# posgraph/coupe.DVSG

Measured on AMD Instinct MI355X. Metric: stabilized frames/sec (1280x720 RGB), higher is better.
Workload: dtype f32

## Files before the change

### coupe/dvsg_amd/_lib.py

```python
import ctypes
import os

_HERE = os.path.dirname(os.path.abspath(__file__))
LIB_PATH = os.environ.get("DVSG_AMD_LIB") or os.path.join(_HERE, "libdvsg_amd.so")
ABI_VERSION = 1

c_float_p = ctypes.POINTER(ctypes.c_float)
_vp = ctypes.c_void_p
_i = ctypes.c_int

SIGNATURES = {
    "dvsg_tps_solve_f32": [_vp, _vp, _i, _i, _i, _vp, _vp],
    "dvsg_tps_solve_checked_f32": [_vp, _vp, _i, _i, _i, _vp, _vp, _vp],
    "dvsg_tps_warp_f32": [_vp, _vp, _vp, _i, _i, _i, _i, _i, _i, _i, _vp, _vp, _vp, _vp],
    "dvsg_flow_warp_f32": [_vp, _vp, _i, _i, _i, _i, _vp, _vp],
    "dvsg_stn_sample_f32": [_vp, _vp, _vp, _i, _i, _i, _i, _i, _i, _vp, _vp],
    "dvsg_grid_affine_f32": [_vp, _vp, _i, _i, _i, _i, _i, _i, _vp, _vp, _vp, _vp],
    "dvsg_grid_projective_f32": [_vp, _vp, _i, _i, _i, _i, _i, _i, _vp, _vp, _vp, _vp],
    "dvsg_elastic_constants_f32": [_i, _vp, _vp],
    "dvsg_grid_elastic_f32": [_vp, _vp, _vp, _i, _vp, _i, _i, _i, _i, _i, _i, _vp, _vp, _vp, _vp],
    "dvsg_scale_rgb_f32": [_vp, _i, _i, _i, _i, _vp, _vp],
    "dvsg_locnet_create": [_i, ctypes.POINTER(ctypes.c_char_p), ctypes.POINTER(_vp),
                           ctypes.POINTER(_i), ctypes.POINTER(ctypes.c_int64), ctypes.POINTER(_vp)],
    "dvsg_locnet_destroy": [_vp],
# ... 51 lines not shown
QUERIES = ("dvsg_abi_version", "dvsg_last_error_string", "dvsg_target_arch")

_lib = None


class DvsgError(RuntimeError):
    pass


def load():
    global _lib
    if _lib is not None:
        return _lib
    if not os.path.isfile(LIB_PATH):
        raise DvsgError(
            "libdvsg_amd.so not found at %s: build it with ./build.sh (hipcc --offload-arch=gfx950). "
            "coupe.dvsg_amd has no CPU or PyTorch fallback." % LIB_PATH)
    lib = ctypes.CDLL(LIB_PATH)
    lib.dvsg_abi_version.restype = ctypes.c_int
    lib.dvsg_last_error_string.restype = ctypes.c_char_p
    lib.dvsg_target_arch.restype = ctypes.c_char_p
    if lib.dvsg_abi_version() != ABI_VERSION:
        raise DvsgError("libdvsg_amd.so ABI %d != expected %d" % (lib.dvsg_abi_version(), ABI_VERSION))
    for name, argtypes in SIGNATURES.items():
        fn = getattr(lib, name)
        fn.argtypes = argtypes
        fn.restype = ctypes.c_int
    _lib = lib
    for env, opt in (("DVSG_CONV_VARIANT", b"conv_variant"), ("DVSG_FUSE_CONV", b"fuse_conv"),
                     ("DVSG_F16_SPLIT", b"f16_split"), ("DVSG_FUSE_SHORTCUT", b"fuse_shortcut"),
                     ("DVSG_CONV1_VARIANT", b"conv1_variant"), ("DVSG_F16_PAIR_MASK", b"f16_pair_mask"),
                     ("DVSG_WIDE16_PACKED", b"wide16_packed"), ("DVSG_WIDE16_AROWS", b"wide16_arows"),
                     ("DVSG_WIDE16_HREUSE", b"wide16_hreuse"), ("DVSG_FUSED_HREUSE", b"fused_hreuse"),
                     ("DVSG_CONCAT_SC", b"concat_sc"), ("DVSG_FLOW_TILED", b"flow_tiled")):
        if os.environ.get(env) and os.environ.get("DVSG_DEBUG") == "1":
            check(lib.dvsg_debug_set_option(opt, int(os.environ[env])), "dvsg_debug_set_option")
    return lib


def check(status, what):
    if status != 0:
        msg = load().dvsg_last_error_string().decode("utf-8", "replace")
        raise DvsgError("%s failed (status %d): %s" % (what, status, msg))


def call(name, *args):
    check(getattr(load(), name)(*args), name)
```

### coupe/dvsg_amd/csrc/cnn_kernels.h

```cpp
#pragma once
#include "common.h"

namespace dvsg {

enum Precision { kF32 = 0, kF16 = 1, kF32S = 2, kF32X = 3 };
inline size_t elem_size(int prec) { return prec == kF16 ? 2 : 4; }

struct ConvGemm {
  int prec;
  const void *x;
  const void *wt;
  const float *bias;
  const void *res;
  void *y;
  int B, H, W, Cin, Ho, Wo, Cout;
  int ksize, stride, pad;
  int res_H, res_W, res_stride;
  int relu;
  int ldx = 0, res_ld = 0, relu_from = -1;
  const void *wt_packed = nullptr;
  const void *wt_packed_a = nullptr;
  const void *wt_packed_h = nullptr;
  int x3 = 0;
  int wsplit = 0;
// ... 11 lines not shown
size_t wide16_packed_bytes(int rows, int Cin, int ksize);
int launch_pack_wide16(const void *wt, void *out, int rows, int Cin, int ksize, int order, hipStream_t s);
void set_wide16_arows(int v);
void set_wide16_hreuse(int v);
void set_wide16_packed(int v);
int launch_zero_tickets(int *tickets, size_t n, hipStream_t s);
struct ConvFused {
  const float *x;
  const float *wt2;
  const float *bias2;
  const float *wt3;
  const float *bias3;
  const float *res;
  float *y;
  int B, H, W, Cin, Ho, Wo, Cout;
  int stride;
  int res_H, res_W, res_stride;
  const float *sc_x = nullptr;
  const float *sc_wt = nullptr;
  const float *sc_bias = nullptr;
  int sc_cin = 0;
  int pieces = 0;
  int f16 = 0;
  int x3 = 0;
};
int launch_conv3x3_1x1_x3(const ConvFused &p, hipStream_t s);
bool conv_fusable(int prec, int Cin, int Cmid, int Cout, int ksize);
int launch_conv3x3_1x1(const ConvFused &p, hipStream_t s);
void set_fuse_conv(int v);
int get_fuse_conv();
void set_fused_hreuse(int v);
void set_conv_variant(int v);
void set_conv1_variant(int v);

constexpr int kConv1Cin = 21;
constexpr int kConv1K = 7 * kConv1Cin;
constexpr int kConv1Kpad = 148;
constexpr int kConv1Ld = 150;
constexpr int kConv1LdH = 168;
constexpr int kConv1X3Ld = 88;
constexpr int kConv1X3StageElems = 3 * 64 * kConv1X3Ld;
enum Conv1SrcKind { kSrcWindow = 0, kSrcRingF32 = 1, kSrcRingU8 = 2 };
struct Conv1Src {
  const void *base;
  const int *table;
  int n_pool;
  const float *mask = nullptr;
};
int launch_conv1(int out_prec, const Conv1Src &src, int src_kind, const float *wt1, const void *wt1h, const void *wt1s,
                 const void *wt1x, const float *bias, void *y, int B, int H, int W, int Ho, int Wo, hipStream_t s);

int launch_maxpool(int prec, const void *x, void *y, int B, int H, int W, int C, int Ho, int Wo, int pad_top,
                   int pad_left, hipStream_t s);

constexpr int kPoolSplits = 8;
int launch_avgpool_partial(int prec, const void *x, float *part, int B, int HW, int C, hipStream_t s);

int launch_f16_to_f32(const void *x, float *y, size_t n, hipStream_t s);
int launch_p_to_f32(const void *x, float *y, size_t n, hipStream_t s);
int launch_f32_to_p(const float *x, void *y, size_t n, hipStream_t s);

constexpr int kDenseSplits = 8;
int launch_dense(const float *xin, int s_in, const float *bias_in, float scale_in, int lrelu_in,
                 const float *W, float *out_part, int B, int K, int N, hipStream_t s);
int launch_dense_finalize(const float *part, int s_in, float scale, const float *bias, float *out, int B,
                          int N, hipStream_t s);

}
```

### coupe/dvsg_amd/csrc/conv1_pool.hip

```cpp
#include <cstdint>
#include <type_traits>

#include "cnn_device.h"
#include "cnn_kernels.h"

namespace dvsg {
namespace {

constexpr int C1_TILE = 128;
constexpr int C1_SEG_PAD = 5488;
constexpr int C1_WELEMS = 64 * kConv1Ld;
constexpr int C1_LDC = 68;

template <int NT, int GROUPS, bool ALIGNED, bool MASKED = false>
struct Conv1Row {
  static constexpr bool kRing = false;
  typedef float floatx4_u __attribute__((ext_vector_type(4), aligned(4)));
  floatx4 nmean[GROUPS];
  long idx[GROUPS];
  unsigned col_ok, full;
  bool fast;
  struct Data {
    floatx4 reg[GROUPS];
    float m0[MASKED ? GROUPS : 1], m1[MASKED ? GROUPS : 1];
// ... 425 lines not shown
  const unsigned long long t_loop_end = C1_STAMP();
#endif
  float *Cs = w_s;
  __syncthreads();
#pragma unroll
  for (int mi = 0; mi < MI; ++mi)
#pragma unroll
    for (int q = 0; q < 16; ++q)
      Cs[(wm * 32 * MI + mi * 32 + (q & 3) + 8 * (q >> 2) + 4 * h) * C1_LDC + wn * 32 + r] = acc[mi][q];
  __syncthreads();
  const int col4 = tid & 15, row0 = tid >> 4;
  const float4 b4 = *reinterpret_cast<const float4 *>(bias + 4 * col4);
  TO *yrow = y + (((size_t)b * Ho + ho) * Wo + wo0) * 64 + 4 * col4;
#pragma unroll 4
  for (int row = row0; row < C1_TILE; row += NT / 16) {
    if (wo0 + row >= Wo) break;
    float4 v = *reinterpret_cast<const float4 *>(Cs + row * C1_LDC + 4 * col4);
    v.x = fmaxf(v.x + b4.x, 0.f);
    v.y = fmaxf(v.y + b4.y, 0.f);
    v.z = fmaxf(v.z + b4.z, 0.f);
    v.w = fmaxf(v.w + b4.w, 0.f);
    store4(yrow + (size_t)row * 64, v);
  }
#ifdef DVSG_STAMPS
  if (tid == 0 && blockIdx.x < 65536) {
    unsigned long long *o = g_c1_stamps + (size_t)blockIdx.x * 8;
    const unsigned long long t_end = C1_STAMP();
    o[0] = st[0]; o[1] = st[1]; o[2] = st[2]; o[3] = st[3]; o[4] = st[4];
    o[5] = t_loop_end - t_begin;
    o[6] = t_end - t_begin;
    o[7] = __builtin_amdgcn_s_memrealtime() - r_begin;
  }
#endif
}

template <typename T>
__global__ __launch_bounds__(256) void maxpool_kernel(const T *__restrict__ x, T *__restrict__ y, int H, int W,
                                                     int C4, int Ho, int Wo, int pad_top, int pad_left,
                                                     size_t total) {
  {
    const size_t e = (size_t)xcd_remap(blockIdx.x, gridDim.x) * 256 + threadIdx.x;
    if (e >= total) return;
    const int c4 = (int)(e % C4);
    size_t t = e / C4;
    const int wo = (int)(t % Wo);
    t /= Wo;
    const int ho = (int)(t % Ho);
    const size_t b = t / Ho;
    float4 m = make_float4(-INFINITY, -INFINITY, -INFINITY, -INFINITY);
#pragma unroll
    for (int i = 0; i < 3; ++i) {
      const int hi = 2 * ho - pad_top + i;
      if (hi < 0 || hi >= H) continue;
#pragma unroll
      for (int j = 0; j < 3; ++j) {
        const int wi = 2 * wo - pad_left + j;
        if (wi < 0 || wi >= W) continue;
        const float4 v = load4(x + (((b * H + hi) * W + wi) * C4 + c4) * 4);
        m.x = fmaxf(m.x, v.x);
        m.y = fmaxf(m.y, v.y);
        m.z = fmaxf(m.z, v.z);
        m.w = fmaxf(m.w, v.w);
      }
    }
    store4(y + e * 4, m);
  }
// ... 964 lines not shown
    if (hi < 0 || hi >= H) continue;
#pragma unroll
    for (int j = 0; j < 3; ++j) {
      const int wi = 2 * wo - pad_left + j;
      if (wi < 0 || wi >= W) continue;
      const float4 v = load4_p(x, (((b * H + hi) * W + wi) * C4 + c4) * 4);
      m.x = fmaxf(m.x, v.x);
      m.y = fmaxf(m.y, v.y);
      m.z = fmaxf(m.z, v.z);
      m.w = fmaxf(m.w, v.w);
    }
  }
  store4_p(y, e * 4, m);
}

int march_bands(int B, int Ho, int wtiles, int *quads_per_band) {
  const int quads = (Ho + C1M_QUAD - 1) / C1M_QUAD;
  const long cols = (long)B * wtiles;
  for (int qpb = 8; qpb >= 4; --qpb) {
    const int bands = (quads + qpb - 1) / qpb;
    if (cols * bands >= 3 * 256) {
      if (quads_per_band) *quads_per_band = qpb;
      return bands;
    }
  }
  return 0;
}

int g_conv1_variant = 0;

}

void set_conv1_variant(int v) { g_conv1_variant = v; }

int launch_conv1(int out_prec, const Conv1Src &src, int src_kind, const float *wt1, const void *wt1h, const void *wt1s,
                 const void *wt1x, const float *bias, void *y, int B, int H, int W, int Ho, int Wo, hipStream_t s) {
  const int wtiles = ceil_div(Wo, C1_TILE);
  const long blocks = (long)wtiles * Ho * B;
  DVSG_REQUIRE(blocks > 0 && blocks < (1L << 31), "conv1: grid of %ld workgroups out of range", blocks);
  DVSG_REQUIRE((long)W * kConv1Cin < (1L << 31), "conv1: input row too long");
  DVSG_REQUIRE(src_kind == kSrcWindow || (src.table && src.n_pool > 0), "conv1: a frame ring needs its index table");
  const double in_bytes = src_kind == kSrcRingU8 ? 1.0 : 4.0;
  ProfScope prof(kClsConv1, s, 2.0 * (double)B * Ho * Wo * 64 * 49 * kConv1Cin,
                 in_bytes * (double)B * H * W * kConv1Cin + (double)elem_size(out_prec) * B * Ho * Wo * 64);
  const dim3 grid((unsigned)blocks);
  const bool aligned = W % 4 == 0 && reinterpret_cast<uintptr_t>(src.base) % (src_kind == kSrcRingU8 ? 4 : 16) == 0;
  const int SRC = 2 * src_kind + (aligned ? 1 : 0) + (src.mask ? 8 : 0);
  if (out_prec == kF32S && !wt1s) return fail(DVSG_ERR_UNSUPPORTED, "conv1: the f32s precision needs the piece weights");
#define DVSG_K_F32(SRC) conv1_kernel<4, float, SRC>
#define DVSG_K_F16(SRC) conv1_f16_kernel<_Float16, (SRC) & 7>
#define DVSG_K_SPLIT(SRC) conv1_split_kernel<float, SRC>
#define DVSG_K_X3(SRC) conv1_x3_kernel<SRC>
#define DVSG_C1(KERNEL, NTHREADS, WPTR, YPTR)                                                                            \
  do {                                                                                                                   \
    switch (SRC) {                                                                                                       \
      case 0: hipLaunchKernelGGL((KERNEL(0)), grid, dim3(NTHREADS), 0, s, src, WPTR, bias, YPTR, H, W, Ho, Wo, wtiles); break; \
      case 1: hipLaunchKernelGGL((KERNEL(1)), grid, dim3(NTHREADS), 0, s, src, WPTR, bias, YPTR, H, W, Ho, Wo, wtiles); break; \
      case 2: hipLaunchKernelGGL((KERNEL(2)), grid, dim3(NTHREADS), 0, s, src, WPTR, bias, YPTR, H, W, Ho, Wo, wtiles); break; \
      case 3: hipLaunchKernelGGL((KERNEL(3)), grid, dim3(NTHREADS), 0, s, src, WPTR, bias, YPTR, H, W, Ho, Wo, wtiles); break; \
      case 4: hipLaunchKernelGGL((KERNEL(4)), grid, dim3(NTHREADS), 0, s, src, WPTR, bias, YPTR, H, W, Ho, Wo, wtiles); break; \
      case 5: hipLaunchKernelGGL((KERNEL(5)), grid, dim3(NTHREADS), 0, s, src, WPTR, bias, YPTR, H, W, Ho, Wo, wtiles); break; \
      case 8: hipLaunchKernelGGL((KERNEL(8)), grid, dim3(NTHREADS), 0, s, src, WPTR, bias, YPTR, H, W, Ho, Wo, wtiles); break; \
      case 9: hipLaunchKernelGGL((KERNEL(9)), grid, dim3(NTHREADS), 0, s, src, WPTR, bias, YPTR, H, W, Ho, Wo, wtiles); break; \
      case 10: hipLaunchKernelGGL((KERNEL(10)), grid, dim3(NTHREADS), 0, s, src, WPTR, bias, YPTR, H, W, Ho, Wo, wtiles); break; \
      case 11: hipLaunchKernelGGL((KERNEL(11)), grid, dim3(NTHREADS), 0, s, src, WPTR, bias, YPTR, H, W, Ho, Wo, wtiles); break; \
      case 12: hipLaunchKernelGGL((KERNEL(12)), grid, dim3(NTHREADS), 0, s, src, WPTR, bias, YPTR, H, W, Ho, Wo, wtiles); break; \
// ... 63 lines not shown
#undef DVSG_K_X3
  return check_launch("conv1_kernel");
}

#ifdef DVSG_STAMPS
extern "C" int dvsg_debug_read_conv1_stamps(void *host, size_t bytes) {
  return hipMemcpyFromSymbol(host, HIP_SYMBOL(g_c1_stamps), bytes) == hipSuccess ? 0 : -3;
}
#endif

int launch_maxpool(int prec, const void *x, void *y, int B, int H, int W, int C, int Ho, int Wo, int pad_top,
                   int pad_left, hipStream_t s) {
  DVSG_REQUIRE(C % 4 == 0 && (prec != kF32S || C % 32 == 0), "maxpool: C=%d must be a multiple of 4 (32 in the f32s format)", C);
  const size_t total = (size_t)B * Ho * Wo * (C / 4);
  const size_t want = (total + 255) / 256;
  DVSG_REQUIRE(want < (1u << 31), "maxpool: %zu blocks do not fit a grid", want);
  const int blocks = (int)want;
  ProfScope prof(kClsMaxpool, s, 0.0, (double)elem_size(prec) * C * ((double)B * H * W + (double)B * Ho * Wo));
  if (prec == kF32S)
    hipLaunchKernelGGL(maxpool_p_kernel, dim3(blocks), dim3(256), 0, s, x, y, H, W, C / 4, Ho, Wo, pad_top, pad_left, total);
  else if (prec == kF16 && C % 8 == 0) {
    const size_t total8 = total / 2;
    hipLaunchKernelGGL(maxpool_h8_kernel, dim3((unsigned)((total8 + 255) / 256)), dim3(256), 0, s, static_cast<const _Float16 *>(x),
                       static_cast<_Float16 *>(y), H, W, C / 8, Ho, Wo, pad_top, pad_left, total8);
  } else if (prec == kF16)
    hipLaunchKernelGGL(maxpool_kernel<_Float16>, dim3(blocks), dim3(256), 0, s, static_cast<const _Float16 *>(x),
                       static_cast<_Float16 *>(y), H, W, C / 4, Ho, Wo, pad_top, pad_left, total);
  else
    hipLaunchKernelGGL(maxpool_kernel<float>, dim3(blocks), dim3(256), 0, s, static_cast<const float *>(x),
                       static_cast<float *>(y), H, W, C / 4, Ho, Wo, pad_top, pad_left, total);
  return check_launch("maxpool_kernel");
}

}
```

### coupe/dvsg_amd/csrc/locnet.hip

```cpp
#include <cmath>
#include <cstring>
#include <map>
#include <string>
#include <vector>

#include "cnn_kernels.h"

namespace dvsg {
namespace {

constexpr float kBnEps = 1e-5f;
const char *kPrefix = "stabNet/localizationNet/";

struct HostArray {
  const float *data;
  int nd;
  int64_t dims[4];
  size_t size() const {
    size_t n = 1;
    for (int i = 0; i < nd; ++i) n *= (size_t)dims[i];
    return n;
  }
};

// ... 248 lines not shown
  if (int rc = upload(net, wts, &L->wt32s)) return rc;
  if (int rc = upload(net, wtx, &L->wt3x)) return rc;
  return upload(net, shift, &L->bias);
}

struct Dims {
  int H1, W1, Hp, Wp, pad_top, pad_left;
};

Dims root_dims(int H, int W) {
  Dims d;
  d.H1 = (H - 1) / 2 + 1;
  d.W1 = (W - 1) / 2 + 1;
  d.Hp = (d.H1 + 1) / 2;
  d.Wp = (d.W1 + 1) / 2;
  const int pth = std::max((d.Hp - 1) * 2 + 3 - d.H1, 0), ptw = std::max((d.Wp - 1) * 2 + 3 - d.W1, 0);
  d.pad_top = pth / 2;
  d.pad_left = ptw / 2;
  return d;
}

size_t align256(size_t n) { return (n + 255) & ~(size_t)255; }

int g_f16_split = 1;
int g_f16_pair_mask = 0xFFFF;
enum LayerKind { kKindC1 = 0, kKindC2 = 1, kKindC3 = 2, kKindSc = 3 };
inline bool f16_pairs(const dvsg_locnet *net, int block, int kind) {
  return g_f16_split && ((g_f16_pair_mask & net->f16_pair_mask) >> (4 * kind + block)) & 1;
}
int g_fuse_shortcut = 1;
int g_x3_conv1 = 1;
int g_x3_fuse = 3;
int g_concat_sc = 1;

struct Workspace {
  char *bufA, *bufB, *bufS, *r1, *r2;
  float *pool_part, *dpart0, *dpart1, *T, *Ft;
  char *splitk_slabs;
  int *splitk_counters;
  size_t total;
};
constexpr int kMaxConvLaunches = 64;

Workspace plan(char *base, int B, int H, int W) {
  const Dims d = root_dims(H, W);
  size_t big_el = std::max((size_t)d.H1 * d.W1 * 64, (size_t)d.Hp * d.Wp * 64);
  size_t small_el = 0;
  {
    int h = d.Hp, w = d.Wp;
    for (const BlockSpec &bs : kBlocks)
      for (int u = 1; u <= bs.units; ++u) {
        const int stride = u == bs.units ? bs.last_stride : 1;
        const int ho = (h - 1) / stride + 1, wo = (w - 1) / stride + 1;
        small_el = std::max(small_el, (size_t)h * w * bs.base);
        big_el = std::max(big_el, (size_t)ho * wo * bs.base * 4);
        if (u == 1) big_el = std::max(big_el, (size_t)h * w * bs.base * 5);
        h = ho; w = wo;
      }
  }
  const size_t big = align256((size_t)B * big_el * sizeof(float));
  const size_t small = align256((size_t)B * small_el * sizeof(float));
  Workspace w;
  size_t off = 0;
  auto take = [&](size_t bytes) {
    char *p = base + off;
    off += align256(bytes);
    return p;
  };
  w.bufA = take(big);
  w.bufB = take(big);
  w.bufS = take(big);
  w.r1 = take(small);
  w.r2 = take(small);
  w.pool_part = reinterpret_cast<float *>(take((size_t)kPoolSplits * B * 2048 * sizeof(float)));
  w.dpart0 = reinterpret_cast<float *>(take((size_t)kDenseSplits * 16 * 2048 * sizeof(float)));
  w.dpart1 = reinterpret_cast<float *>(take((size_t)kDenseSplits * 16 * 2048 * sizeof(float)));
  w.T = reinterpret_cast<float *>(take((size_t)B * 2 * 28 * sizeof(float)));
  w.Ft = reinterpret_cast<float *>(take((size_t)B * 50 * sizeof(float)));
  w.splitk_slabs = take(kSplitKSlabBytes);
  w.splitk_counters = reinterpret_cast<int *>(take((size_t)kMaxConvLaunches * kSplitKMaxTiles * sizeof(int)));
  w.total = off;
  return w;
}

int run_conv(int prec, const ConvLayer &L, bool pairs, const void *x, int B, int H, int W, void *y, int Ho, int Wo,
             const void *res, int res_H, int res_W, int res_stride, bool relu, const Workspace &ws, int *launch_idx,
             hipStream_t s, int ldx = 0, int res_ld = 0, int relu_from = -1) {
  ConvGemm p;
  p.ldx = ldx; p.res_ld = res_ld; p.relu_from = relu_from;
  p.splitk_scratch = ws.splitk_slabs;
  p.splitk_scratch_bytes = kSplitKSlabBytes;
  p.splitk_counters = ws.splitk_counters + (size_t)((*launch_idx)++ % kMaxConvLaunches) * kSplitKMaxTiles;
  p.prec = prec == kF32S || prec == kF32X ? kF32 : prec;
  p.wsplit = prec == kF32S || (prec == kF16 && pairs);
  p.x3 = prec == kF32X;
  if (prec == kF32X && !L.wt3x)
    return fail(DVSG_ERR_UNSUPPORTED, "f32x3: layer %d -> %d (k = %d) has no packed bfloat16 pieces (K %% 32, Cout %% 64)", L.cin, L.cout, L.ksize);
  p.x = x; p.wt = L.weights(prec, p.wsplit != 0); p.bias = L.bias; p.res = res; p.y = y;
  if (prec == kF16 && pairs) {
    p.wt_packed = L.wt16p;
    p.wt_packed_a = L.wt16pa;
// ... 57 lines not shown
    return fail(DVSG_ERR_WORKSPACE, "locnet forward: workspace %zu bytes < required %zu", workspace_bytes, ws.total);
  const Dims d = root_dims(H, W);
  const int gprec = prec;
  if (prec == kF32X) prec = kF32;

  auto tap = [&](int stage, const void *act, int h, int w, int c) -> int {
    if (stage != stop_stage) return 0;
    const size_t n = (size_t)B * h * w * c;
    if (n * sizeof(float) > act_out_bytes)
      return fail(DVSG_ERR_INVALID_ARG, "tap buffer %zu bytes < %zu", act_out_bytes, n * sizeof(float));
    if (prec == kF16) {
      if (int rc = launch_f16_to_f32(act, act_out, n, s)) return rc;
    } else if (prec == kF32S) {
      if (int rc = launch_p_to_f32(act, act_out, n, s)) return rc;
    } else {
      DVSG_HIP(hipMemcpyAsync(act_out, act, n * sizeof(float), hipMemcpyDeviceToDevice, s));
    }
    act_dims[0] = h; act_dims[1] = w; act_dims[2] = c;
    return 1;
  };
#define DVSG_TAP(stage, act, h, w, c)          \
  do {                                         \
    int t_ = tap(stage, act, h, w, c);         \
    if (t_ < 0) return t_;                     \
    if (t_ > 0) return DVSG_OK;                \
  } while (0)
#define DVSG_RUN(call)             \
  do {                             \
    if (int rc_ = (call)) return rc_; \
  } while (0)

  DVSG_RUN(launch_zero_tickets(ws.splitk_counters, (size_t)kMaxConvLaunches * kSplitKMaxTiles, s));
  int launch_idx = 0;
  {
  MarkerRange mr("dvsg/conv1");
  DVSG_RUN(launch_conv1(gprec == kF32X && g_x3_conv1 ? kF32X : prec, src, src_kind, net->conv1.wt, net->conv1.wt16, net->conv1.wt32s,
                        net->conv1.wt3x, net->conv1.bias, ws.bufA, B, H, W, d.H1, d.W1, s));
  }
  DVSG_TAP(0, ws.bufA, d.H1, d.W1, 64);
  {
  MarkerRange mr("dvsg/pool1");
  DVSG_RUN(launch_maxpool(prec, ws.bufA, ws.bufB, B, d.H1, d.W1, 64, d.Hp, d.Wp, d.pad_top, d.pad_left, s));
  }
  DVSG_TAP(1, ws.bufB, d.Hp, d.Wp, 64);

  char *X = ws.bufB, *Y = ws.bufA;
  int h = d.Hp, w = d.Wp;
  int stage = 2;
  int unit_in_block = 0, last_block = -1;
  for (const Unit &u : net->units) {
    unit_in_block = u.block == last_block ? unit_in_block + 1 : 1;
    last_block = u.block;
    char range_name[40];
    std::snprintf(range_name, sizeof(range_name), "dvsg/block%d/unit_%d", u.block + 1, unit_in_block);
    MarkerRange mr(range_name);
    const int ho = (h - 1) / u.stride + 1, wo = (w - 1) / u.stride + 1;
    const void *res = X;
    int res_h = h, res_w = w, res_stride = u.stride;
    const int calib_slot = 3 * (stage - 2);
    DVSG_RUN(calib_record(calib_slot, X, (long)B * h * w, u.c1.cin, s));
    const bool x3_fused = gprec == kF32X && g_x3_fuse == 3;
    const bool x3_unfused = gprec == kF32X && (g_x3_fuse == 0 || (g_x3_fuse == 1 && !u.has_shortcut));
    const bool fuse23 = !x3_unfused && conv_fusable(prec, u.c2.cin, u.c2.cout, u.c3.cout, u.c2.ksize) &&
                        (prec != kF16 || (f16_pairs(net, u.block, kKindC2) && f16_pairs(net, u.block, kKindC3) &&
                                          (!u.has_shortcut || f16_pairs(net, u.block, kKindSc))));
    const bool fuse_sc = fuse23 && !x3_fused && u.has_shortcut && u.stride == 1 && u.shortcut.cin == 64 && u.shortcut.cout == 256 &&
                         g_fuse_shortcut;
    const bool cat = u.has_shortcut && !fuse_sc && u.has_cat && prec != kF16 && g_concat_sc && !g_calib.on && u.stride == 1;
    const void *c2_in = ws.r1;
    int c2_ldx = 0, res_ld = 0;
    if (cat) {
      DVSG_RUN(run_conv(gprec, u.cat, false, X, B, h, w, ws.bufS, h, w, nullptr, 0, 0, 1, false, ws, &launch_idx, s, 0, 0,
                        u.shortcut.cout));
      res = ws.bufS;
      res_h = ho; res_w = wo; res_stride = 1;
// ... 461 lines not shown
  }
  if (std::strcmp(name, "wide16_arows") == 0) {
    set_wide16_arows(value);
    return DVSG_OK;
  }
  if (std::strcmp(name, "wide16_packed") == 0) {
    set_wide16_packed(value);
    return DVSG_OK;
  }
  if (std::strcmp(name, "flow_tiled") == 0) {
    set_flow_tiled(value);
    return DVSG_OK;
  }
  if (std::strcmp(name, "flow_rounds") == 0) {
    set_flow_rounds(value);
    return DVSG_OK;
  }
  if (std::strcmp(name, "warp_xcd") == 0) {
    set_warp_xcd(value);
    return DVSG_OK;
  }
  if (std::strcmp(name, "conv1_variant") == 0) {
    set_conv1_variant(value);
    return DVSG_OK;
  }
  if (std::strcmp(name, "fuse_conv") == 0) {
    set_fuse_conv(value);
    return DVSG_OK;
  }
  if (std::strcmp(name, "concat_sc") == 0) {
    g_concat_sc = value != 0;
    return DVSG_OK;
  }
  if (std::strcmp(name, "x3_conv1") == 0) {
    g_x3_conv1 = value;
    return DVSG_OK;
  }
  if (std::strcmp(name, "x3_fuse") == 0) {
    g_x3_fuse = value;
    return DVSG_OK;
  }
  if (std::strcmp(name, "fuse_shortcut") == 0) {
    g_fuse_shortcut = value != 0;
    return DVSG_OK;
  }
  if (std::strcmp(name, "f16_split") == 0) {
    g_f16_split = value != 0;
    return DVSG_OK;
  }
  if (std::strcmp(name, "f16_pair_mask") == 0) {
    g_f16_pair_mask = value & 0xFFFF;
    return DVSG_OK;
  }
  return fail(DVSG_ERR_INVALID_ARG, "dvsg_debug_set_option: unknown option %s", name);
}

static int calibrate_f16(dvsg_locnet *net, const float *patches, int B, int H, int W, int mode, void *workspace,
                         size_t workspace_bytes, hipStream_t s) {
  std::vector<double> mu((size_t)48 * 2048, 1.0);
  if (mode == 2) {
    void *sums = nullptr, *part = nullptr, *F = nullptr;
    hipError_t e = hipMalloc(&sums, 48 * 2048 * sizeof(double));
    if (e == hipSuccess) e = hipMalloc(&part, (size_t)kCalibBlocks * 2048 * sizeof(float));
    if (e == hipSuccess) e = hipMalloc(&F, (size_t)B * 50 * sizeof(float));
    if (e == hipSuccess) e = hipMemsetAsync(sums, 0, 48 * 2048 * sizeof(double), s);
    int rc = e == hipSuccess ? DVSG_OK : fail(DVSG_ERR_HIP, "calibration: %s", hipGetErrorString(e));
// ... 185 lines not shown
```

Baseline: 743.8.

## Fuse conv1 with 3x3/2 maxpool via banded tiles and seam fixup kernel

Adds a conv1 kernel that max-pools its output tile in shared memory before writing, so the full-resolution conv1 activation never goes to global memory. There are single-group and paired-group (512-thread) variants. Each workgroup covers a band of pooled rows and a strip of columns. Partial maxima at band and strip edges go to side buffers, and a small seams kernel merges them afterwards. With default settings the fused path runs only for f32 conv1, window sources without a mask, and large enough grids; otherwise the separate conv1 and maxpool path is kept. The cost is an extra launch and recomputed boundary rows.

Result: faster. 752.3 (median of 6 runs) (+1.1%).

```diff
diff --git a/coupe/dvsg_amd/_lib.py b/coupe/dvsg_amd/_lib.py
--- a/coupe/dvsg_amd/_lib.py
+++ b/coupe/dvsg_amd/_lib.py
@@ -107,7 +107,9 @@
                      ("DVSG_CONV1_VARIANT", b"conv1_variant"), ("DVSG_F16_PAIR_MASK", b"f16_pair_mask"),
                      ("DVSG_WIDE16_PACKED", b"wide16_packed"), ("DVSG_WIDE16_AROWS", b"wide16_arows"),
                      ("DVSG_WIDE16_HREUSE", b"wide16_hreuse"), ("DVSG_FUSED_HREUSE", b"fused_hreuse"),
-                     ("DVSG_CONCAT_SC", b"concat_sc"), ("DVSG_FLOW_TILED", b"flow_tiled")):
+                     ("DVSG_CONCAT_SC", b"concat_sc"), ("DVSG_FLOW_TILED", b"flow_tiled"),
+                     ("DVSG_CONV1_POOL_FUSED", b"conv1_pool_fused"), ("DVSG_CONV1_POOL_BAND", b"conv1_pool_band"),
+                     ("DVSG_CONV1_POOL_PAIR", b"conv1_pool_pair")):
         if os.environ.get(env) and os.environ.get("DVSG_DEBUG") == "1":
             check(lib.dvsg_debug_set_option(opt, int(os.environ[env])), "dvsg_debug_set_option")
     return lib
diff --git a/coupe/dvsg_amd/csrc/cnn_kernels.h b/coupe/dvsg_amd/csrc/cnn_kernels.h
--- a/coupe/dvsg_amd/csrc/cnn_kernels.h
+++ b/coupe/dvsg_amd/csrc/cnn_kernels.h
@@ -67,6 +67,7 @@
 void set_fused_hreuse(int v);
 void set_conv_variant(int v);
 void set_conv1_variant(int v);
+int get_conv1_variant();
 
 constexpr int kConv1Cin = 21;
 constexpr int kConv1K = 7 * kConv1Cin;
@@ -85,6 +86,10 @@
 int launch_conv1(int out_prec, const Conv1Src &src, int src_kind, const float *wt1, const void *wt1h, const void *wt1s,
                  const void *wt1x, const float *bias, void *y, int B, int H, int W, int Ho, int Wo, hipStream_t s);
 
+void conv1_pool_geometry(int B, int Hp, int Wp, int pband, int *strips, int *bands, size_t *side_elems);
+int launch_conv1_pool(const Conv1Src &src, int src_kind, const float *wt1, const float *bias, float *y, float *side, int B, int H,
+                      int W, int H1, int W1, int Hp, int Wp, int pad_top, int pad_left, int pband, bool pair, hipStream_t s);
+
 int launch_maxpool(int prec, const void *x, void *y, int B, int H, int W, int C, int Ho, int Wo, int pad_top,
                    int pad_left, hipStream_t s);
 
diff --git a/coupe/dvsg_amd/csrc/conv1_pool.hip b/coupe/dvsg_amd/csrc/conv1_pool.hip
--- a/coupe/dvsg_amd/csrc/conv1_pool.hip
+++ b/coupe/dvsg_amd/csrc/conv1_pool.hip
@@ -481,6 +481,423 @@
     o[7] = __builtin_amdgcn_s_memrealtime() - r_begin;
   }
 #endif
+}
+
+constexpr int C1P_Q = C1_TILE / 2;
+constexpr int C1P_TOP = C1P_Q + 1;
+
+template <int SRC>
+__global__ __launch_bounds__(256) __attribute__((amdgpu_waves_per_eu(2, 2)))
+void conv1_pool_kernel(const Conv1Src src, const float *__restrict__ wt1, const float *__restrict__ bias,
+                       float *__restrict__ y, float *__restrict__ side_top, float *__restrict__ side_left, int H, int W,
+                       int H1, int W1, int Hp, int Wp, int pad_top, int pad_left, int strips, int bands, int pband) {
+  constexpr int NT = 256;
+  constexpr int MI = 2;
+  constexpr int IN4 = (C1_SEG_PAD / 4 + NT - 1) / NT;
+  constexpr int WLOADS = (C1_WELEMS / 4 + NT - 1) / NT;
+  const int ROWS = 2 * pband;
+  static_assert(C1_TILE * C1_LDC <= C1_WELEMS, "pool tile must fit in the weight stage");
+  __shared__ __attribute__((aligned(16))) float w_s[C1_WELEMS];
+  __shared__ __attribute__((aligned(16))) float in_s[C1_SEG_PAD];
+  const int tid = threadIdx.x;
+  const int lane = tid & 63, wave = tid >> 6;
+  const int wm = wave >> 1, wn = wave & 1;
+  const int r = lane & 31, h = lane >> 5;
+
+  int blk = xcd_remap(blockIdx.x, gridDim.x);
+  const int s = blk % strips;
+  blk /= strips;
+  const int k = blk % bands;
+  const int b = blk / bands;
+  const int c0 = s * C1_TILE - pad_left;
+  const int r0 = 2 * pband * k - pad_top;
+  const int p0 = pband * k;
+
+  typedef typename Conv1RowSel<NT, IN4, SRC>::type Row;
+  Row row;
+  row.init(src, tid, b, c0, H, W, C1_SEG_PAD);
+  if constexpr (Row::kRing) {
+    for (int e = tid; e < C1_SEG_PAD; e += NT) in_s[e] = 0.f;
+  }
+  typename Row::Data rd;
+  floatx4 w_reg[WLOADS];
+  auto load_stage = [&](int t) __attribute__((always_inline)) {
+    const int j = t / 7, kh = t - 7 * j;
+    row.load(rd, 2 * (r0 + j) + kh - 3);
+    const floatx4 *wsrc = reinterpret_cast<const floatx4 *>(wt1 + (size_t)kh * C1_WELEMS);
+#pragma unroll
+    for (int i = 0; i < WLOADS; ++i) {
+      const int q = tid + NT * i;
+      w_reg[i] = wsrc[q < C1_WELEMS / 4 ? q : 0];
+    }
+  };
+  auto store_stage = [&]() __attribute__((always_inline)) {
+    if constexpr (Row::kRing) {
+      row.scatter(rd, [&](int e, float v) __attribute__((always_inline)) { in_s[e] = v; });
+    } else {
+#pragma unroll
+      for (int i = 0; i < IN4; ++i) {
+        const int q = tid + NT * i;
+        const floatx4 v = row.scaled(rd, i);
+        if (q < C1_SEG_PAD / 4) reinterpret_cast<floatx4 *>(in_s)[q] = v;
+      }
+    }
+#pragma unroll
+    for (int i = 0; i < WLOADS; ++i) {
+      const int q = tid + NT * i;
+      if (q < C1_WELEMS / 4) reinterpret_cast<floatx4 *>(w_s)[q] = w_reg[i];
+    }
+  };
+
+  const float bias_c = bias[wn * 32 + r];
+  float *Cs = w_s;
+  auto pool_out = [&](const floatx16 (&v)[MI], float *dst, long dst_stride, int qofs, float *col0) __attribute__((always_inline)) {
+    __syncthreads();
+#pragma unroll
+    for (int mi = 0; mi < MI; ++mi)
+#pragma unroll
+      for (int q = 0; q < 16; ++q)
+        Cs[(wm * 32 * MI + mi * 32 + (q & 3) + 8 * (q >> 2) + 4 * h) * C1_LDC + wn * 32 + r] = v[mi][q];
+    __syncthreads();
+    const int col4 = tid & 15;
+    if (col0 && tid < 16) store4(col0 + 4 * col4, *reinterpret_cast<const float4 *>(Cs + 4 * col4));
+#pragma unroll
+    for (int qq = tid >> 4; qq < C1P_Q; qq += NT / 16) {
+      if (s * C1P_Q + qq >= Wp) break;
+      float4 m = make_float4(-INFINITY, -INFINITY, -INFINITY, -INFINITY);
+#pragma unroll
+      for (int j = 0; j < 3; ++j) {
+        const int c = 2 * qq + j;
+        if (c >= C1_TILE || c0 + c < 0 || c0 + c >= W1) continue;
+        const float4 x = *reinterpret_cast<const float4 *>(Cs + c * C1_LDC + 4 * col4);
+        m.x = fmaxf(m.x, x.x);
+        m.y = fmaxf(m.y, x.y);
+        m.z = fmaxf(m.z, x.z);
+        m.w = fmaxf(m.w, x.w);
+      }
+      store4(dst + (long)(qofs + qq) * dst_stride + 4 * col4, m);
+    }
+  };
+
+  floatx16 acc[MI], vmax[MI];
+#pragma unroll
+  for (int mi = 0; mi < MI; ++mi)
+#pragma unroll
+    for (int q = 0; q < 16; ++q) acc[mi][q] = 0.f;
+
+  load_stage(0);
+#pragma unroll 1
+  for (int j = 0; j < ROWS; ++j) {
+#pragma unroll 1
+    for (int kh = 0; kh < 7; ++kh) {
+      __syncthreads();
+      store_stage();
+      __syncthreads();
+      if (7 * j + kh + 1 < 7 * ROWS) load_stage(7 * j + kh + 1);
+      __builtin_amdgcn_sched_barrier(0);
+      const float *a0 = in_s + 2 * kConv1Cin * (wm * 32 * MI + r) + 2 * h;
+      const float *bp = w_s + (wn * 32 + r) * kConv1Ld + 2 * h;
+      constexpr int STEPS = kConv1Kpad / 4, PAIRS = (STEPS + 1) / 2;
+      float2 va[2][2][MI], vb[2][2];
+      auto read_pair = [&](int slot, int g) __attribute__((always_inline)) {
+#pragma unroll
+        for (int jj = 0; jj < 2; ++jj) {
+          if (2 * g + jj >= STEPS) break;
+#pragma unroll
+          for (int mi = 0; mi < MI; ++mi)
+            va[slot][jj][mi] = *reinterpret_cast<const float2 *>(a0 + mi * (2 * kConv1Cin * 32) + 4 * (2 * g + jj));
+          vb[slot][jj] = *reinterpret_cast<const float2 *>(bp + 4 * (2 * g + jj));
+        }
+      };
+      read_pair(0, 0);
+#pragma unroll
+      for (int g = 0; g < PAIRS; ++g) {
+        if (g + 1 < PAIRS) read_pair((g + 1) & 1, g + 1);
+        __builtin_amdgcn_sched_barrier(0);
+#pragma unroll
+        for (int jj = 0; jj < 2; ++jj) {
+          if (2 * g + jj >= STEPS) break;
+#pragma unroll
+          for (int mi = 0; mi < MI; ++mi) acc[mi] = mfma32(va[g & 1][jj][mi].x, vb[g & 1][jj].x, acc[mi]);
+#pragma unroll
+          for (int mi = 0; mi < MI; ++mi) acc[mi] = mfma32(va[g & 1][jj][mi].y, vb[g & 1][jj].y, acc[mi]);
+        }
+        __builtin_amdgcn_sched_barrier(0);
+      }
+    }
+    const int cr = r0 + j;
+    const bool row_ok = cr >= 0 && cr < H1;
+#pragma unroll
+    for (int mi = 0; mi < MI; ++mi)
+#pragma unroll
+      for (int q = 0; q < 16; ++q) acc[mi][q] = row_ok ? fmaxf(acc[mi][q] + bias_c, 0.f) : -INFINITY;
+    if (j == 0) {
+      if (k > 0) {
+        float *rec = side_top + (((size_t)b * bands + k) * strips + s) * (C1P_TOP * 64);
+        pool_out(acc, rec + 64, 64, 0, s > 0 ? rec : nullptr);
+      }
+#pragma unroll
+      for (int mi = 0; mi < MI; ++mi) vmax[mi] = acc[mi];
+    } else if (j & 1) {
+#pragma unroll
+      for (int mi = 0; mi < MI; ++mi)
+#pragma unroll
+        for (int q = 0; q < 16; ++q) vmax[mi][q] = fmaxf(vmax[mi][q], acc[mi][q]);
+    } else {
+#pragma unroll
+      for (int mi = 0; mi < MI; ++mi)
+#pragma unroll
+        for (int q = 0; q < 16; ++q) vmax[mi][q] = fmaxf(vmax[mi][q], acc[mi][q]);
+      const int p = p0 + j / 2 - 1;
+      if (p < Hp)
+        pool_out(vmax, y + ((size_t)b * Hp + p) * Wp * 64, 64, s * C1P_Q,
+                 s > 0 ? side_left + (((size_t)b * Hp + p) * strips + s) * 64 : nullptr);
+#pragma unroll
+      for (int mi = 0; mi < MI; ++mi) vmax[mi] = acc[mi];
+    }
+#pragma unroll
+    for (int mi = 0; mi < MI; ++mi)
+#pragma unroll
+      for (int q = 0; q < 16; ++q) acc[mi][q] = 0.f;
+  }
+  const int p = p0 + pband - 1;
+  if (p < Hp)
+    pool_out(vmax, y + ((size_t)b * Hp + p) * Wp * 64, 64, s * C1P_Q,
+             s > 0 ? side_left + (((size_t)b * Hp + p) * strips + s) * 64 : nullptr);
+}
+
+template <int SRC>
+__global__ __launch_bounds__(512) __attribute__((amdgpu_waves_per_eu(2, 2)))
+void conv1_pool_pair_kernel(const Conv1Src src, const float *__restrict__ wt1, const float *__restrict__ bias,
+                            float *__restrict__ y, float *__restrict__ side_top, float *__restrict__ side_left, int H, int W,
+                            int H1, int W1, int Hp, int Wp, int pad_top, int pad_left, int strips, int bands, int pband) {
+  constexpr int NT = 512, NG = 256;
+  constexpr int MI = 2;
+  constexpr int IN4 = (C1_SEG_PAD / 4 + NG - 1) / NG;
+  constexpr int WLOADS = (C1_WELEMS / 4 + NT - 1) / NT;
+  static_assert(C1_TILE * C1_LDC <= C1_WELEMS && C1_TILE * C1_LDC <= 2 * C1_SEG_PAD, "pool tiles must fit in the idle stages");
+  __shared__ __attribute__((aligned(16))) float w_s[C1_WELEMS];
+  __shared__ __attribute__((aligned(16))) float in_s[2 * C1_SEG_PAD];
+  const int tid = threadIdx.x;
+  const int grp = tid >> 8, gt = tid & (NG - 1);
+  const int lane = tid & 63, wave = (tid >> 6) & 3;
+  const int wm = wave >> 1, wn = wave & 1;
+  const int r = lane & 31, h = lane >> 5;
+  float *seg = in_s + grp * C1_SEG_PAD;
+
+  int blk = xcd_remap(blockIdx.x, gridDim.x);
+  const int s = blk % strips;
+  blk /= strips;
+  const int k = blk % bands;
+  const int b = blk / bands;
+  const int c0 = s * C1_TILE - pad_left;
+  const int r0 = 2 * pband * k - pad_top;
+  const int p0 = pband * k;
+
+  typedef typename Conv1RowSel<NG, IN4, SRC>::type Row;
+  Row row;
+  row.init(src, gt, b, c0, H, W, C1_SEG_PAD);
+  auto zero_segments = [&]() __attribute__((always_inline)) {
+    for (int e = tid; e < 2 * C1_SEG_PAD; e += NT) in_s[e] = 0.f;
+  };
+  if constexpr (Row::kRing) zero_segments();
+  typename Row::Data rd;
+  floatx4 w_reg[WLOADS];
+  auto load_stage = [&](int t) __attribute__((always_inline)) {
+    const int i = t / 7, kh = t - 7 * i;
+    row.load(rd, 2 * (r0 + 2 * i + grp) + kh - 3);
+    const floatx4 *wsrc = reinterpret_cast<const floatx4 *>(wt1 + (size_t)kh * C1_WELEMS);
+#pragma unroll
+    for (int j = 0; j < WLOADS; ++j) {
+      const int q = tid + NT * j;
+      w_reg[j] = wsrc[q < C1_WELEMS / 4 ? q : 0];
+    }
+  };
+  auto store_stage = [&]() __attribute__((always_inline)) {
+    if constexpr (Row::kRing) {
+      row.scatter(rd, [&](int e, float v) __attribute__((always_inline)) { seg[e] = v; });
+    } else {
+#pragma unroll
+      for (int j = 0; j < IN4; ++j) {
+        const int q = gt + NG * j;
+        const floatx4 v = row.scaled(rd, j);
+        if (q < C1_SEG_PAD / 4) reinterpret_cast<floatx4 *>(seg)[q] = v;
+      }
+    }
+#pragma unroll
+    for (int j = 0; j < WLOADS; ++j) {
+      const int q = tid + NT * j;
+      if (q < C1_WELEMS / 4) reinterpret_cast<floatx4 *>(w_s)[q] = w_reg[j];
+    }
+  };
+
+  const float bias_c = bias[wn * 32 + r];
+  float *Cs = grp ? in_s : w_s;
+  floatx16 acc[MI], prev[MI];
+  auto emit = [&](int mode, bool both, float *dst, int qofs, float *col0) __attribute__((always_inline)) {
+    __syncthreads();
+    if (grp == 0 || both) {
+#pragma unroll
+      for (int mi = 0; mi < MI; ++mi)
+#pragma unroll
+        for (int q = 0; q < 16; ++q) {
+          const float v = mode == 0 ? acc[mi][q] : (mode == 1 && grp == 0 ? fmaxf(prev[mi][q], acc[mi][q]) : prev[mi][q]);
+          Cs[(wm * 32 * MI + mi * 32 + (q & 3) + 8 * (q >> 2) + 4 * h) * C1_LDC + wn * 32 + r] = v;
+        }
+    }
+    __syncthreads();
+    const int col4 = tid & 15;
+    auto tile4 = [&](int c) __attribute__((always_inline)) {
+      float4 x = *reinterpret_cast<const float4 *>(w_s + c * C1_LDC + 4 * col4);
+      if (both) {
+        const float4 o = *reinterpret_cast<const float4 *>(in_s + c * C1_LDC + 4 * col4);
+        x.x = fmaxf(x.x, o.x);
+        x.y = fmaxf(x.y, o.y);
+        x.z = fmaxf(x.z, o.z);
+        x.w = fmaxf(x.w, o.w);
+      }
+      return x;
+    };
+    if (col0 && tid < 16) store4(col0 + 4 * col4, tile4(0));
+#pragma unroll
+    for (int qq = tid >> 4; qq < C1P_Q; qq += NT / 16) {
+      if (s * C1P_Q + qq >= Wp) break;
+      float4 m = make_float4(-INFINITY, -INFINITY, -INFINITY, -INFINITY);
+#pragma unroll
+      for (int j = 0; j < 3; ++j) {
+        const int c = 2 * qq + j;
+        if (c >= C1_TILE || c0 + c < 0 || c0 + c >= W1) continue;
+        const float4 x = tile4(c);
+        m.x = fmaxf(m.x, x.x);
+        m.y = fmaxf(m.y, x.y);
+        m.z = fmaxf(m.z, x.z);
+        m.w = fmaxf(m.w, x.w);
+      }
+      store4(dst + (long)(qofs + qq) * 64 + 4 * col4, m);
+    }
+    if constexpr (Row::kRing) {
+      __syncthreads();
+      zero_segments();
+    }
+  };
+
+#pragma unroll
+  for (int mi = 0; mi < MI; ++mi)
+#pragma unroll
+    for (int q = 0; q < 16; ++q) acc[mi][q] = 0.f;
+
+  load_stage(0);
+#pragma unroll 1
+  for (int i = 0; i < pband; ++i) {
+#pragma unroll 1
+    for (int kh = 0; kh < 7; ++kh) {
+      __syncthreads();
+      store_stage();
+      __syncthreads();
+      if (7 * i + kh + 1 < 7 * pband) load_stage(7 * i + kh + 1);
+      __builtin_amdgcn_sched_barrier(0);
+      const float *a0 = seg + 2 * kConv1Cin * (wm * 32 * MI + r) + 2 * h;
+      const float *bp = w_s + (wn * 32 + r) * kConv1Ld + 2 * h;
+      constexpr int STEPS = kConv1Kpad / 4, PAIRS = (STEPS + 1) / 2;
+      float2 va[2][2][MI], vb[2][2];
+      auto read_pair = [&](int slot, int g) __attribute__((always_inline)) {
+#pragma unroll
+        for (int jj = 0; jj < 2; ++jj) {
+          if (2 * g + jj >= STEPS) break;
+#pragma unroll
+          for (int mi = 0; mi < MI; ++mi)
+            va[slot][jj][mi] = *reinterpret_cast<const float2 *>(a0 + mi * (2 * kConv1Cin * 32) + 4 * (2 * g + jj));
+          vb[slot][jj] = *reinterpret_cast<const float2 *>(bp + 4 * (2 * g + jj));
+        }
+      };
+      read_pair(0, 0);
+#pragma unroll
+      for (int g = 0; g < PAIRS; ++g) {
+        if (g + 1 < PAIRS) read_pair((g + 1) & 1, g + 1);
+        __builtin_amdgcn_sched_barrier(0);
+#pragma unroll
+        for (int jj = 0; jj < 2; ++jj) {
+          if (2 * g + jj >= STEPS) break;
+#pragma unroll
+          for (int mi = 0; mi < MI; ++mi) acc[mi] = mfma32(va[g & 1][jj][mi].x, vb[g & 1][jj].x, acc[mi]);
+#pragma unroll
+          for (int mi = 0; mi < MI; ++mi) acc[mi] = mfma32(va[g & 1][jj][mi].y, vb[g & 1][jj].y, acc[mi]);
+        }
+        __builtin_amdgcn_sched_barrier(0);
+      }
+    }
+    const int cr = r0 + 2 * i + grp;
+    const bool row_ok = cr >= 0 && cr < H1;
+#pragma unroll
+    for (int mi = 0; mi < MI; ++mi)
+#pragma unroll
+      for (int q = 0; q < 16; ++q) acc[mi][q] = row_ok ? fmaxf(acc[mi][q] + bias_c, 0.f) : -INFINITY;
+    if (i == 0) {
+      if (k > 0) {
+        float *rec = side_top + (((size_t)b * bands + k) * strips + s) * (C1P_TOP * 64);
+        emit(0, false, rec + 64, 0, s > 0 ? rec : nullptr);
+      }
+    } else {
+      const int p = p0 + i - 1;
+      if (p < Hp)
+        emit(1, true, y + ((size_t)b * Hp + p) * Wp * 64, s * C1P_Q,
+             s > 0 ? side_left + (((size_t)b * Hp + p) * strips + s) * 64 : nullptr);
+    }
+#pragma unroll
+    for (int mi = 0; mi < MI; ++mi) {
+      prev[mi] = acc[mi];
+#pragma unroll
+      for (int q = 0; q < 16; ++q) acc[mi][q] = 0.f;
+    }
+  }
+  const int p = p0 + pband - 1;
+  if (p < Hp)
+    emit(2, true, y + ((size_t)b * Hp + p) * Wp * 64, s * C1P_Q,
+         s > 0 ? side_left + (((size_t)b * Hp + p) * strips + s) * 64 : nullptr);
+}
+
+__global__ __launch_bounds__(256) void conv1_pool_seams_kernel(float *__restrict__ y, const float *__restrict__ side_top,
+                                                               const float *__restrict__ side_left, int B, int Hp, int Wp,
+                                                               int strips, int bands, int pband, long n_a, long n_b) {
+  long e = (long)blockIdx.x * 256 + threadIdx.x;
+  if (e >= n_a + n_b) return;
+  const int c4 = (int)(e & 15);
+  auto vmax4 = [](float4 &m, const float *p) {
+    const float4 x = *reinterpret_cast<const float4 *>(p);
+    m.x = fmaxf(m.x, x.x);
+    m.y = fmaxf(m.y, x.y);
+    m.z = fmaxf(m.z, x.z);
+    m.w = fmaxf(m.w, x.w);
+  };
+  if (e < n_a) {
+    long t = e >> 4;
+    const int q = (int)(t % Wp);
+    t /= Wp;
+    const int kk = 1 + (int)(t % (bands - 1));
+    const int b = (int)(t / (bands - 1));
+    const int p = pband * kk - 1;
+    const int s = q / C1P_Q, qq = q - s * C1P_Q;
+    float *out = y + (((size_t)b * Hp + p) * Wp + q) * 64 + 4 * c4;
+    float4 m = *reinterpret_cast<const float4 *>(out);
+    vmax4(m, side_top + ((((size_t)b * bands + kk) * strips + s) * C1P_TOP + 1 + qq) * 64 + 4 * c4);
+    if (qq == C1P_Q - 1 && s + 1 < strips) {
+      vmax4(m, side_left + (((size_t)b * Hp + p) * strips + s + 1) * 64 + 4 * c4);
+      vmax4(m, side_top + (((size_t)b * bands + kk) * strips + s + 1) * C1P_TOP * 64 + 4 * c4);
+    }
+    store4(out, m);
+  } else {
+    long t = (e - n_a) >> 4;
+    const int s = (int)(t % (strips - 1));
+    t /= strips - 1;
+    const int p = (int)(t % Hp);
+    const int b = (int)(t / Hp);
+    if (p % pband == pband - 1 && p / pband + 1 < bands) return;
+    const int q = (s + 1) * C1P_Q - 1;
+    float *out = y + (((size_t)b * Hp + p) * Wp + q) * 64 + 4 * c4;
+    float4 m = *reinterpret_cast<const float4 *>(out);
+    vmax4(m, side_left + (((size_t)b * Hp + p) * strips + s + 1) * 64 + 4 * c4);
+    store4(out, m);
+  }
 }
 
 template <typename T>
@@ -1511,6 +1928,7 @@
 }
 
 void set_conv1_variant(int v) { g_conv1_variant = v; }
+int get_conv1_variant() { return g_conv1_variant; }
 
 int launch_conv1(int out_prec, const Conv1Src &src, int src_kind, const float *wt1, const void *wt1h, const void *wt1s,
                  const void *wt1x, const float *bias, void *y, int B, int H, int W, int Ho, int Wo, hipStream_t s) {
@@ -1640,4 +2058,59 @@
   return check_launch("maxpool_kernel");
 }
 
+
+void conv1_pool_geometry(int B, int Hp, int Wp, int pband, int *strips, int *bands, size_t *side_elems) {
+  const int st = ceil_div(Wp, C1P_Q), bd = ceil_div(Hp, pband);
+  if (strips) *strips = st;
+  if (bands) *bands = bd;
+  if (side_elems) *side_elems = (size_t)B * bd * st * C1P_TOP * 64 + (size_t)B * Hp * st * 64;
 }
+
+int launch_conv1_pool(const Conv1Src &src, int src_kind, const float *wt1, const float *bias, float *y, float *side, int B, int H,
+                      int W, int H1, int W1, int Hp, int Wp, int pad_top, int pad_left, int pband, bool pair, hipStream_t s) {
+  DVSG_REQUIRE(pband >= 1, "conv1_pool: %d pooled rows per band", pband);
+  DVSG_REQUIRE(pad_top >= 0 && pad_top <= 1 && pad_left >= 0 && pad_left <= 1, "conv1_pool: pads %d, %d out of range", pad_top,
+               pad_left);
+  DVSG_REQUIRE(Hp == (H1 + 1) / 2 && Wp == (W1 + 1) / 2, "conv1_pool: pooled size %dx%d is not 3x3/2 SAME of %dx%d", Hp, Wp, H1, W1);
+  DVSG_REQUIRE((long)W * kConv1Cin < (1L << 31), "conv1: input row too long");
+  DVSG_REQUIRE(src_kind == kSrcWindow || (src.table && src.n_pool > 0), "conv1: a frame ring needs its index table");
+  int strips = 0, bands = 0;
+  size_t side_elems = 0;
+  conv1_pool_geometry(B, Hp, Wp, pband, &strips, &bands, &side_elems);
+  const long blocks = (long)strips * bands * B;
+  DVSG_REQUIRE(blocks > 0 && blocks < (1L << 31), "conv1_pool: grid of %ld workgroups out of range", blocks);
+  float *side_top = side, *side_left = side + (size_t)B * bands * strips * C1P_TOP * 64;
+  const double in_bytes = src_kind == kSrcRingU8 ? 1.0 : 4.0;
+  {
+    ProfScope prof(kClsConv1, s, 2.0 * (double)B * H1 * W1 * 64 * 49 * kConv1Cin,
+                   in_bytes * (double)B * H * W * kConv1Cin + 4.0 * B * Hp * Wp * 64);
+    const bool aligned = pad_left == 0 && W % 4 == 0 &&
+                         reinterpret_cast<uintptr_t>(src.base) % (src_kind == kSrcRingU8 ? 4 : 16) == 0;
+    const int SRC = 2 * src_kind + (aligned ? 1 : 0) + (src.mask ? 8 : 0);
+    const dim3 grid((unsigned)blocks);
+#define DVSG_CP(S)                                                                                                         \
+  case S:                                                                                                                  \
+    if (pair)                                                                                                              \
+      hipLaunchKernelGGL((conv1_pool_pair_kernel<S>), grid, dim3(512), 0, s, src, wt1, bias, y, side_top, side_left, H, W, H1, \
+                         W1, Hp, Wp, pad_top, pad_left, strips, bands, pband);                                             \
+    else                                                                                                                   \
+      hipLaunchKernelGGL((conv1_pool_kernel<S>), grid, dim3(256), 0, s, src, wt1, bias, y, side_top, side_left, H, W, H1, W1, \
+                         Hp, Wp, pad_top, pad_left, strips, bands, pband);                                                 \
+    break
+    switch (SRC) {
+      DVSG_CP(0); DVSG_CP(1); DVSG_CP(2); DVSG_CP(3); DVSG_CP(4); DVSG_CP(5);
+      DVSG_CP(8); DVSG_CP(9); DVSG_CP(10); DVSG_CP(11); DVSG_CP(12); DVSG_CP(13);
+      default: return fail(DVSG_ERR_INVALID_ARG, "conv1_pool: source kind %d", SRC);
+    }
+#undef DVSG_CP
+    if (int rc = check_launch("conv1_pool_kernel")) return rc;
+  }
+  const long n_a = (long)B * (bands - 1) * Wp * 16, n_b = (long)B * Hp * (strips - 1) * 16;
+  if (n_a + n_b == 0) return DVSG_OK;
+  ProfScope prof(kClsMaxpool, s, 0.0, 4.0 * 64 * ((double)B * (bands - 1) * Wp * 3 + (double)B * Hp * (strips - 1) * 2));
+  hipLaunchKernelGGL(conv1_pool_seams_kernel, dim3((unsigned)((n_a + n_b + 255) / 256)), dim3(256), 0, s, y, side_top, side_left, B,
+                     Hp, Wp, strips, bands, pband, n_a, n_b);
+  return check_launch("conv1_pool_seams_kernel");
+}
+
+}
diff --git a/coupe/dvsg_amd/csrc/locnet.hip b/coupe/dvsg_amd/csrc/locnet.hip
--- a/coupe/dvsg_amd/csrc/locnet.hip
+++ b/coupe/dvsg_amd/csrc/locnet.hip
@@ -304,9 +304,15 @@
 int g_x3_conv1 = 1;
 int g_x3_fuse = 3;
 int g_concat_sc = 1;
+int g_conv1_pool_fused = -1;
+constexpr int kConv1PoolBand = 3;
+int g_conv1_pool_band = 0;
+int g_conv1_pool_pair = 1;
+constexpr long kConv1PoolMinBlocks = 4 * 512;
 
 struct Workspace {
   char *bufA, *bufB, *bufS, *r1, *r2;
+  size_t big;
   float *pool_part, *dpart0, *dpart1, *T, *Ft;
   char *splitk_slabs;
   int *splitk_counters;
@@ -339,6 +345,7 @@
     off += align256(bytes);
     return p;
   };
+  w.big = big;
   w.bufA = take(big);
   w.bufB = take(big);
   w.bufS = take(big);
@@ -462,15 +469,30 @@
 
   DVSG_RUN(launch_zero_tickets(ws.splitk_counters, (size_t)kMaxConvLaunches * kSplitKMaxTiles, s));
   int launch_idx = 0;
+  const int c1prec = gprec == kF32X && g_x3_conv1 ? kF32X : prec;
+  int strips = 0, bands = 0;
+  size_t side_elems = 0;
+  const int pband = g_conv1_pool_band > 0 ? g_conv1_pool_band : kConv1PoolBand;
+  conv1_pool_geometry(B, d.Hp, d.Wp, pband, &strips, &bands, &side_elems);
+  const bool pool_fused = c1prec == kF32 && stop_stage != 0 && get_conv1_variant() == 0 && g_conv1_pool_fused != 0 &&
+                          side_elems * sizeof(float) <= ws.big &&
+                          (g_conv1_pool_fused == 1 ||
+                           (src_kind == kSrcWindow && !src.mask && (long)B * strips * bands >= kConv1PoolMinBlocks));
+  if (pool_fused) {
+    MarkerRange mr("dvsg/conv1");
+    DVSG_RUN(launch_conv1_pool(src, src_kind, net->conv1.wt, net->conv1.bias, reinterpret_cast<float *>(ws.bufB),
+                               reinterpret_cast<float *>(ws.bufA), B, H, W, d.H1, d.W1, d.Hp, d.Wp, d.pad_top, d.pad_left, pband, g_conv1_pool_pair != 0, s));
+  } else {
   {
   MarkerRange mr("dvsg/conv1");
-  DVSG_RUN(launch_conv1(gprec == kF32X && g_x3_conv1 ? kF32X : prec, src, src_kind, net->conv1.wt, net->conv1.wt16, net->conv1.wt32s,
+  DVSG_RUN(launch_conv1(c1prec, src, src_kind, net->conv1.wt, net->conv1.wt16, net->conv1.wt32s,
                         net->conv1.wt3x, net->conv1.bias, ws.bufA, B, H, W, d.H1, d.W1, s));
   }
   DVSG_TAP(0, ws.bufA, d.H1, d.W1, 64);
   {
   MarkerRange mr("dvsg/pool1");
   DVSG_RUN(launch_maxpool(prec, ws.bufA, ws.bufB, B, d.H1, d.W1, 64, d.Hp, d.Wp, d.pad_top, d.pad_left, s));
+  }
   }
   DVSG_TAP(1, ws.bufB, d.Hp, d.Wp, 64);
 
@@ -998,6 +1020,18 @@
     g_concat_sc = value != 0;
     return DVSG_OK;
   }
+  if (std::strcmp(name, "conv1_pool_fused") == 0) {
+    g_conv1_pool_fused = value;
+    return DVSG_OK;
+  }
+  if (std::strcmp(name, "conv1_pool_pair") == 0) {
+    g_conv1_pool_pair = value;
+    return DVSG_OK;
+  }
+  if (std::strcmp(name, "conv1_pool_band") == 0) {
+    g_conv1_pool_band = value;
+    return DVSG_OK;
+  }
   if (std::strcmp(name, "x3_conv1") == 0) {
     g_x3_conv1 = value;
     return DVSG_OK;
```
